# samuel-watson/glmmrMCML

Hardware: AMD Instinct MI355X
Metric: MCML iters/sec x m chains (simlik evals/sec) (higher is better)
Workload: dtype f64

## Files before the change

### glmmrmcml_amd/_lib.py

```python
import ctypes as C
import os
import re

_HERE = os.path.dirname(os.path.abspath(__file__))
LIB_PATH = os.environ.get("GLMMR_MCML_LIB") or os.path.join(_HERE, "libglmmr_mcml_hip.so")
HEADER_PATH = os.path.join(os.path.dirname(_HERE), "include", "glmmr_mcml_c.h")
_lib = None


class McmlError(RuntimeError):
    def __init__(self, code, msg):
        super().__init__("glmmr_mcml error %d: %s" % (code, msg))
        self.code = code


_RETURNS = {"int": C.c_int, "long long": C.c_longlong, "const char*": C.c_char_p}
_SCALARS = {"int": C.c_int, "double": C.c_double, "long long": C.c_longlong, "uint64_t": C.c_uint64, "uint32_t": C.c_uint32}
_CALLBACKS = ("glmmr_mcml_objective", "glmmr_mcml_batch_objective", "glmmr_mcml_parts_objective")
_DECL = re.compile(r"(?<=[;{}]) ?([\w ]+?\*?) ?\b(glmmr_mcml_\w+) ?\(([^()]*)\) ?;")


def prototypes(header):
    text = re.sub(r"/\*.*?\*/", " ", header, flags=re.S)
    text = " ".join(re.sub(r"^\s*#.*$", "", text, flags=re.M).split())
# ... 16 lines not shown

def lib():
    global _lib
    if _lib is None:
        if not os.path.exists(LIB_PATH):
            raise ImportError(
                "%s not built: run `python -c 'import __graft_entry__ as g; g.build()'` "
                "(hipcc --offload-arch=gfx950); glmmrmcml_amd has no CPU fallback" % LIB_PATH)
        if not os.path.exists(HEADER_PATH):
            raise ImportError("%s is missing: the prototypes of %s are read from it" % (HEADER_PATH, LIB_PATH))
        L = C.CDLL(LIB_PATH)
        with open(HEADER_PATH) as f:
            for name, (restype, argtypes) in prototypes(f.read()).items():
                fn = getattr(L, name)
                fn.restype, fn.argtypes = restype, argtypes
        _lib = L
    return _lib


def check(rc):
    if rc != 0:
        raise McmlError(rc, lib().glmmr_mcml_last_error().decode(errors="replace"))
```

### glmmrmcml_amd/csrc/band_plan.h

```cpp
#pragma once
#include "common.h"
#include <algorithm>
#include <map>
#include <memory>

namespace mcml {

constexpr int BD_BM = 80, BD_BN = 128, BD_BK = 32, BD_STAGES = 3;
constexpr int BD_A_BYTES = BD_BK * BD_BM * 8;
constexpr int BD_B_BYTES = BD_BK * BD_BN * 8;
constexpr int BD_STAGE_BYTES = BD_A_BYTES + BD_B_BYTES;
constexpr size_t BD_LDS_BYTES = (size_t)BD_STAGES * BD_STAGE_BYTES;
constexpr int BD_NA = 3, BD_NB = 4, BD_PER_TILE = BD_NA + BD_NB;
constexpr int BD_TILE_ELEMS = BD_BM * BD_BN;

struct BandItem { int band, kt0, kt1, slot; };
struct BandRed { int band, s0, s1, pad; };

struct BandPlanDev {
    int gn = 0, nwg = 0, nred = 0, nslots = 0;
    int paired = 0;
    DevBuf items, wg_ptr, red, part;
};

struct SkinnyPlan {
    int nrb = 0, nkc = 0, ldp = 0;
    DevBuf range;
    DevBuf part;
};

struct BandPlan {
    int M = 0, K = 0, nbands = 0;
    std::vector<int> kr;
    long tiles = 0;
    std::map<int, std::unique_ptr<BandPlanDev>> by_gn;
    std::unique_ptr<SkinnyPlan> skinny;

    void reset(int M_, int K_, const std::vector<int>& kr_)
    {
        M = M_; K = K_; kr = kr_; nbands = (M + BD_BM - 1) / BD_BM;
        tiles = 0;
        for (int b = 0; b < nbands; ++b) tiles += kr[2 * b + 1] - kr[2 * b];
        by_gn.clear();
        skinny.reset();
    }

    static bool decompose(const std::vector<int>& kr, int nbands, int gn, int target_wg, std::vector<BandItem>& items,
                          std::vector<int>& wg_ptr, std::vector<BandRed>& red, int& nslots)
    {
        items.clear(); wg_ptr.clear(); red.clear(); nslots = 0;
        constexpr long OVH = 3;
        const int npairs = (nbands + 1) / 2;
        if ((long)npairs * gn * 5 >= (long)target_wg * 4) {
            auto cost = [&](int b) { return 2L * (kr[2 * b + 1] - kr[2 * b]) + OVH; };
            int G = target_wg / gn; if (G > nbands) G = nbands; if (G < 1) G = 1;
            std::vector<int> order(nbands);
            for (int b = 0; b < nbands; ++b) order[b] = b;
            std::stable_sort(order.begin(), order.end(), [&](int a, int b) { return cost(a) > cost(b); });
            std::vector<long> load(G, 0);
            std::vector<std::vector<int>> group(G);
            for (int b : order) {
                const int g = (int)(std::min_element(load.begin(), load.end()) - load.begin());
                group[g].push_back(b); load[g] += cost(b);
            }
            long pair_max = 0;
            for (int p = 0; p < npairs; ++p)
                pair_max = std::max(pair_max, cost(p) + (nbands - 1 - p > p ? cost(nbands - 1 - p) : 0));
            auto waves = [&](int groups) { return ((long)groups * gn + target_wg - 1) / target_wg; };
            if (waves(npairs) * pair_max < waves(G) * *std::max_element(load.begin(), load.end())) {
                group.assign(npairs, std::vector<int>());
                for (int p = 0; p < npairs; ++p) {
                    group[p].push_back(p);
                    if (nbands - 1 - p > p) group[p].push_back(nbands - 1 - p);
                }
            }
            for (std::vector<int>& g : group) {
                std::sort(g.begin(), g.end());
                wg_ptr.push_back((int)items.size());
                for (int b : g) items.push_back({b, kr[2 * b], kr[2 * b + 1], -1});
            }
            wg_ptr.push_back((int)items.size());
            return true;
        }
        int nwg = target_wg / gn; if (nwg < 1) nwg = 1;
        auto fill = [&](long cap, bool emit) -> int {
            int used = 1; long room = cap;
            if (emit) wg_ptr.push_back(0);
            for (int b = 0; b < nbands; ++b) {
                int k0 = kr[2 * b]; const int k1 = kr[2 * b + 1];
                const int first = (int)items.size();
                int pieces = 0;
                do {
                    if (room < OVH + 2) { ++used; room = cap; if (emit) wg_ptr.push_back((int)items.size()); }
                    long take = (room - OVH) / 2; if (take > k1 - k0) take = k1 - k0;
                    if (emit) items.push_back({b, k0, k0 + (int)take, -1});
                    k0 += (int)take; room -= OVH + 2 * take; ++pieces;
                } while (k0 < k1);
                if (emit && pieces > 1) {
                    for (int t = 0; t < pieces; ++t) items[first + t].slot = nslots + t;
                    red.push_back({b, nslots, nslots + pieces, 0});
                    nslots += pieces;
                }
            }
            if (emit) wg_ptr.push_back((int)items.size());
            return used;
        };
        long T = 0;
        for (int b = 0; b < nbands; ++b) T += kr[2 * b + 1] - kr[2 * b];
        long lo = OVH + 2, hi = 2 * T + OVH * nbands + OVH + 2;
        while (lo < hi) {
            const long mid = (lo + hi) / 2;
            if (fill(mid, false) <= nwg) hi = mid; else lo = mid + 1;
        }
        fill(lo, true);
        return false;
    }

    int device_plan(int gn, hipStream_t s, BandPlanDev** out)
    {
        auto it = by_gn.find(gn);
        if (it != by_gn.end()) { *out = it->second.get(); return MCML_OK; }
        std::unique_ptr<BandPlanDev> d(new BandPlanDev());
        std::vector<BandItem> items; std::vector<int> wg_ptr; std::vector<BandRed> red; int nslots = 0;
        d->paired = decompose(kr, nbands, gn, 256, items, wg_ptr, red, nslots) ? 1 : 0;
        d->gn = gn; d->nwg = (int)wg_ptr.size() - 1; d->nred = (int)red.size(); d->nslots = nslots;
        MCML_TRY(d->items.ensure(sizeof(BandItem) * (items.size() + 1)));
        MCML_TRY(d->wg_ptr.ensure(sizeof(int) * wg_ptr.size()));
        MCML_HIP(hipMemcpyAsync(d->items.p, items.data(), sizeof(BandItem) * items.size(), hipMemcpyHostToDevice, s));
        MCML_HIP(hipMemcpyAsync(d->wg_ptr.p, wg_ptr.data(), sizeof(int) * wg_ptr.size(), hipMemcpyHostToDevice, s));
        if (nslots > 0) {
            MCML_TRY(d->red.ensure(sizeof(BandRed) * red.size()));
            MCML_HIP(hipMemcpyAsync(d->red.p, red.data(), sizeof(BandRed) * red.size(), hipMemcpyHostToDevice, s));
            MCML_TRY(d->part.ensure(sizeof(double) * (size_t)nslots * gn * BD_TILE_ELEMS));
        }
        MCML_HIP(hipStreamSynchronize(s));
        *out = d.get();
        by_gn[gn] = std::move(d);
        return MCML_OK;
    }
};

}
```

### glmmrmcml_amd/csrc/cabi.hip

```cpp
#include "entry.h"
#include "hmc_chain.h"
#include <atomic>

using namespace mcml;

struct Mode {
    int Ctx::*field;
    const char* env;
    const char* names[4];
    const char* valid;
    std::atomic<int> dflt{-1};

    int get()
    {
        if (dflt.load() < 0) {
            const char* e = getenv(env);
            int unset = -1, m = 0;
            for (int i = 1; e && names[i]; ++i) if (!strcmp(e, names[i])) m = i;
            dflt.compare_exchange_strong(unset, m);
        }
        return dflt.load();
    }
    int check(const char* fn, bool ok, int mode) const
    {
// ... 322 lines not shown
{
    return m <= 0 ? 0 : sample_shape(m, 0, chains).ncols;
}

extern "C" int glmmr_mcml_ctx_profile(glmmr_mcml_ctx* h, int enable, int reset, double* out8)
{
    MCML_REQUIRE(h, "profile: null context");
    Ctx& c = h->c;
    KernelProf& p = c.prof;
    if (out8) {
        out8[0] = p.ms[0]; out8[1] = (double)p.cnt[0]; out8[2] = p.ms[1]; out8[3] = (double)p.cnt[1];
        const double C = (double)c.hmc.C, dense = 2.0 * c.n * (double)c.Q * C;
        double ff = dense, fb = dense, kind = 0;
        if (c.sp.active) { ff = fb = 2.0 * (double)c.sp.nnz * C; kind = 2; }
        else {
            if (c.band_fwd) { ff = 2.0 * 80.0 * 32.0 * (double)c.band_fwd_tiles * C; kind = 1; }
            if (c.band_bwd) { fb = 2.0 * 80.0 * 32.0 * (double)c.band_bwd_tiles * C; kind = 1; }
        }
        out8[4] = ff; out8[5] = fb; out8[6] = dense; out8[7] = kind;
    }
    if (reset) for (int i = 0; i < 4; ++i) { p.ms[i] = 0; p.cnt[i] = 0; p.seen[i] = 0; }
    if (enable && !p.on) {
        MCML_HIP(hipSetDevice(c.device));
        while (p.ev.size() < 4096) { hipEvent_t e; if (hipEventCreate(&e) != hipSuccess) { (void)hipGetLastError(); break; } p.ev.push_back(e); }
    }
    p.on = enable != 0;
    return MCML_OK;
}

extern "C" int glmmr_mcml_ctx_profile_launches(glmmr_mcml_ctx* h, long long* fwd, long long* bwd)
{
    MCML_REQUIRE(h, "profile_launches: null context");
// ... 319 lines not shown
```

### glmmrmcml_amd/csrc/ctx_hooks.hip

```cpp
#include "entry.h"
#include "sparse_plan.h"
#include <algorithm>

using namespace mcml;

extern "C" int glmmr_mcml_dbg_theta_log(glmmr_mcml_ctx* h, int enable, double* out, int cap_rows, int* nrows)
{
    MCML_REQUIRE(h, "theta_log: null context");
    Ctx& c = h->c;
    const int w = c.cov.npar + 1;
    const int have = (int)(c.theta_log.size() / (size_t)w);
    if (nrows) *nrows = have;
    if (out) {
        const int take = have < cap_rows ? have : cap_rows;
        memcpy(out, c.theta_log.data() + (size_t)(have - take) * w, sizeof(double) * (size_t)take * w);
        if (nrows) *nrows = take;
    }
    if (enable >= 0) { c.theta_log_on = enable != 0; if (enable) c.theta_log.clear(); }
    return MCML_OK;
}

extern "C" int glmmr_mcml_dbg_band_plan(glmmr_mcml_ctx* h, int which, int chains, int* out10)
{
    MCML_REQUIRE(h && (which == 0 || which == 1) && chains >= 1 && out10, "dbg_band_plan: bad argument");
    const Ctx& c = h->c;
    const BandPlan& bp = which ? c.plan_bwd : c.plan_fwd;
    const int gn = (chains + BD_BN - 1) / BD_BN;
    if (c.sp.active) {
        for (int i = 0; i < 10; ++i) out10[i] = 0;
        out10[3] = gn;
        return MCML_OK;
    }
    int nempty = 0;
    for (int b = 0; b < bp.nbands; ++b) nempty += bp.kr[2 * b] == bp.kr[2 * b + 1];
    int nwg = 0, nred = 0, nslots = 0, paired = 0, built = 0;
    auto it = bp.by_gn.find(gn);
    if (it != bp.by_gn.end()) {
        const BandPlanDev& d = *it->second;
        nwg = d.nwg; nred = d.nred; nslots = d.nslots; paired = d.paired; built = 1;
    } else if (bp.nbands > 0) {
        std::vector<BandItem> items; std::vector<int> wg_ptr; std::vector<BandRed> red;
        paired = BandPlan::decompose(bp.kr, bp.nbands, gn, 256, items, wg_ptr, red, nslots) ? 1 : 0;
        nwg = (int)wg_ptr.size() - 1; nred = (int)red.size();
    }
    const int v[10] = {(which ? c.band_bwd : c.band_fwd) ? 1 : 0, bp.nbands, (int)bp.tiles, gn, nwg, nred, nslots,
                       paired, nempty, built};
    for (int i = 0; i < 10; ++i) out10[i] = v[i];
    return MCML_OK;
}

extern "C" int glmmr_mcml_dbg_sparse_plan(glmmr_mcml_ctx* h, int chains, long long* out12)
{
    MCML_REQUIRE(h && chains >= 1 && out12, "dbg_sparse_plan: bad argument");
    const Ctx& c = h->c;
    const SparseZL& sp = c.sp;
    for (int i = 0; i < 12; ++i) out12[i] = 0;
    out12[0] = sp.active ? 1 : 0;
    out12[10] = cm_qrows(c.Q); out12[11] = cm_chain_blocks(chains);
    if (!sp.active) return MCML_OK;
    out12[1] = sp.factored ? 1 : 0; out12[2] = sp.W; out12[3] = sp.nnz; out12[4] = sp.nnz_z; out12[5] = sp.nnz_l;
    out12[6] = sp.nblk; out12[7] = sp.max_blk; out12[8] = cm_long_rows(c) ? 1 : 0; out12[9] = cm_fuse_width(c);
    return MCML_OK;
// ... 207 lines not shown
```

### glmmrmcml_amd/csrc/debug_hooks.hip

```cpp
#include "dgemm_mfma.h"
#include "dgemm_dl.h"
#include "dgemm_band.h"

using namespace mcml;

extern "C" int glmmr_mcml_dbg_dgemm(int M, int N, int K, const double* A, int lda,
                                    const double* B, int ldb, int b_nmajor,
                                    double alpha, double beta, double* C, int ldc,
                                    int lower_only, int force_tile)
{
    int ndev = 0;
    if (hipGetDeviceCount(&ndev) != hipSuccess || ndev == 0) {
        set_error("no HIP device: libglmmr_mcml_hip has no CPU fallback");
        return MCML_ENODEVICE;
    }
    hipStream_t s = nullptr;
    DevMat dA, dB, dC;
    if (force_tile == 40) {
        MCML_REQUIRE(!b_nmajor && !lower_only, "dbg_dgemm: the direct-to-LDS kernel takes a K-major B and all tiles");
        const int kpad = round_up(K, 32);
        MCML_TRY(dA.alloc(M, K, 32));
        MCML_HIP(hipMemset(dA.d(), 0, sizeof(double) * (size_t)dA.ld * dA.cols_alloc));
        MCML_HIP(hipMemcpy2D(dA.d(), sizeof(double) * dA.ld, A, sizeof(double) * lda, sizeof(double) * M, K, hipMemcpyHostToDevice));
        MCML_TRY(dB.alloc(kpad, N));
// ... 89 lines not shown
    MCML_HIP(hipEventCreate(&e0));
    MCML_HIP(hipEventCreate(&e1));
    MCML_HIP(hipEventRecord(e0, s));
    for (int i = 0; i < iters; i++) MCML_TRY(go());
    MCML_HIP(hipEventRecord(e1, s));
    MCML_HIP(hipEventSynchronize(e1));
    float ms = 0;
    MCML_HIP(hipEventElapsedTime(&ms, e0, e1));
    *ms_per_launch = ms / iters;
    (void)hipEventDestroy(e0);
    (void)hipEventDestroy(e1);
    return MCML_OK;
}

static int dbg_dgemm_band(int M, int N, int K, const double* A, int lda, const double* B, int ldb, double* C, int ldc,
                          int* tiles_executed, int form, int* whole_band);

extern "C" int glmmr_mcml_dbg_dgemm_band(int M, int N, int K, const double* A, int lda, const double* B, int ldb,
                                         double* C, int ldc, int* tiles_executed)
{
    return dbg_dgemm_band(M, N, K, A, lda, B, ldb, C, ldc, tiles_executed, BAND_FORM_AUTO, nullptr);
}

extern "C" int glmmr_mcml_dbg_dgemm_band_form(int M, int N, int K, const double* A, int lda, const double* B, int ldb,
                                              double* C, int ldc, int* tiles_executed, int form, int* whole_band)
{
    MCML_REQUIRE(form == BAND_FORM_8WAVE || form == BAND_FORM_FEED, "dbg_dgemm_band_form: form is 0 or 1");
    return dbg_dgemm_band(M, N, K, A, lda, B, ldb, C, ldc, tiles_executed, form, whole_band);
}

static int dbg_dgemm_band(int M, int N, int K, const double* A, int lda, const double* B, int ldb, double* C, int ldc,
                          int* tiles_executed, int form, int* whole_band)
{
    int ndev = 0;
    if (hipGetDeviceCount(&ndev) != hipSuccess || ndev == 0) {
        set_error("no HIP device: libglmmr_mcml_hip has no CPU fallback");
        return MCML_ENODEVICE;
    }
    MCML_REQUIRE(M > 0 && N > 0 && K > 0 && A && B && C, "dbg_dgemm_band: bad argument");
    hipStream_t s = nullptr;
    DevMat dA, dB, dC;
    MCML_TRY(dA.alloc(M, K, 32));
    MCML_HIP(hipMemset(dA.d(), 0, sizeof(double) * (size_t)dA.ld * dA.cols_alloc));
    MCML_HIP(hipMemcpy2D(dA.d(), sizeof(double) * dA.ld, A, sizeof(double) * lda, sizeof(double) * M, K, hipMemcpyHostToDevice));
    MCML_TRY(dB.alloc(round_up(K, 32), N));
    MCML_HIP(hipMemset(dB.d(), 0, sizeof(double) * (size_t)dB.ld * N));
    MCML_HIP(hipMemcpy2D(dB.d(), sizeof(double) * dB.ld, B, sizeof(double) * ldb, sizeof(double) * K, N, hipMemcpyHostToDevice));
    MCML_TRY(dC.alloc(M, N));
    MCML_HIP(hipMemset(dC.d(), 0, sizeof(double) * (size_t)dC.ld * N));
    MCML_REQUIRE(dlds_applicable(M, N, K, dA.d(), dA.ld, dA.cols_alloc, dB.d(), dB.ld), "dbg_dgemm_band: contract");
    const int nbands = (M + BD_BM - 1) / BD_BM;
    DevBuf kr;
    MCML_TRY(kr.ensure(sizeof(int) * 2 * nbands));
    hipLaunchKernelGGL(k_band_ranges, dim3(nbands), dim3(256), 0, s, dA.d(), dA.ld, M, K, kr.as<int>());
    MCML_HIP(hipGetLastError());
    std::vector<int> hk(2 * nbands);
    MCML_HIP(hipMemcpy(hk.data(), kr.p, sizeof(int) * 2 * nbands, hipMemcpyDeviceToHost));
    BandPlan plan;
    plan.reset(M, K, hk);
    if (tiles_executed) *tiles_executed = (int)plan.tiles;
    EpiAxpby epi{dC.d(), dC.ld, 1.0, 0.0};
    MCML_TRY(launch_gemm_band(s, plan, N, dA.d(), dA.ld, dB.d(), dB.ld, epi, nullptr, 0, form, whole_band));
    MCML_TRY(download_matrix(C, ldc, dC.d(), dC.ld, M, N, s));
    return MCML_OK;
}

extern "C" int glmmr_mcml_dbg_band_clocks(int M, int N, int iters, int mode, double* out3)
{
    MCML_REQUIRE(mode < 0 || !(mode & 15),
                 "dbg_band_clocks: modes 1, 2, 4 and 8 (the K loop with parts switched off) were retired by the commit "
                 "'Band HMC products: one K-loop pipeline under both kernel forms'; their findings are in DESIGN.md 5.1");
    int ndev = 0;
    if (hipGetDeviceCount(&ndev) != hipSuccess || ndev == 0) {
        set_error("no HIP device: libglmmr_mcml_hip has no CPU fallback");
        return MCML_ENODEVICE;
// ... 3 lines not shown
    std::vector<double> hA((size_t)M * M, 0.0), hB((size_t)M * N);
    uint64_t x = 88172645463325252ULL;
    auto rnd = [&]() { x ^= x << 13; x ^= x >> 7; x ^= x << 17; return (double)(x >> 11) / 9007199254740992.0 * 2 - 1; };
    const bool cst = getenv("GLMMR_MCML_DBG_DATA") && !strcmp(getenv("GLMMR_MCML_DBG_DATA"), "const");
    const bool dec = getenv("GLMMR_MCML_DBG_DATA") && !strcmp(getenv("GLMMR_MCML_DBG_DATA"), "decay");
    for (int j = 0; j < M; ++j) for (int i = j; i < M; ++i) hA[i + (size_t)j * M] = cst ? 1.0 : dec ? rnd() * std::exp(-(double)(i - j) / 40.0) : rnd();
    for (auto& v : hB) v = cst ? 1.0 : rnd();
    DevMat dA, dB, dC;
    MCML_TRY(dA.alloc(M, M, 32));
    MCML_HIP(hipMemset(dA.d(), 0, sizeof(double) * (size_t)dA.ld * dA.cols_alloc));
    MCML_HIP(hipMemcpy2D(dA.d(), sizeof(double) * dA.ld, hA.data(), sizeof(double) * M, sizeof(double) * M, M, hipMemcpyHostToDevice));
    MCML_TRY(dB.alloc(round_up(M, 32), N));
    MCML_HIP(hipMemset(dB.d(), 0, sizeof(double) * (size_t)dB.ld * N));
    MCML_HIP(hipMemcpy2D(dB.d(), sizeof(double) * dB.ld, hB.data(), sizeof(double) * M, sizeof(double) * M, N, hipMemcpyHostToDevice));
    MCML_TRY(dC.alloc(M, N));
    const int nbands = (M + BD_BM - 1) / BD_BM;
    DevBuf kr, clk;
    MCML_TRY(kr.ensure(sizeof(int) * 2 * nbands));
    MCML_TRY(clk.ensure(16));
    MCML_HIP(hipMemset(clk.p, 0, 16));
    hipLaunchKernelGGL(k_band_ranges, dim3(nbands), dim3(256), 0, s, dA.d(), dA.ld, M, M, kr.as<int>());
    std::vector<int> hk(2 * nbands);
    MCML_HIP(hipMemcpy(hk.data(), kr.p, sizeof(int) * 2 * nbands, hipMemcpyDeviceToHost));
    BandPlan plan;
    plan.reset(M, M, hk);
    const double tiles = (double)plan.tiles;
    EpiAxpby epi{dC.d(), dC.ld, 1.0, 0.0};
    if (mode < 0) {
        for (int i = 0; i < 3; i++)
            MCML_TRY((launch_gemm_band<EpiAxpby, false>(s, plan, N, dA.d(), dA.ld, dB.d(), dB.ld, epi)));
        hipEvent_t f0, f1;
        MCML_HIP(hipEventCreate(&f0));
        MCML_HIP(hipEventCreate(&f1));
        MCML_HIP(hipEventRecord(f0, s));
        for (int i = 0; i < iters; i++)
            MCML_TRY((launch_gemm_band<EpiAxpby, false>(s, plan, N, dA.d(), dA.ld, dB.d(), dB.ld, epi)));
        MCML_HIP(hipEventRecord(f1, s));
        MCML_HIP(hipEventSynchronize(f1));
        float fms = 0;
        MCML_HIP(hipEventElapsedTime(&fms, f0, f1));
        out3[0] = fms / iters; out3[1] = 0;
// ... 221 lines not shown
```

### glmmrmcml_amd/csrc/dgemm_band.h

```cpp
#pragma once
#include "dgemm_dlds.h"
#include "band_plan.h"

namespace mcml {

struct BandP {
    GemmP g;
    const BandItem* items;
    const int* wg_ptr;
    int nwg;
    double* part;
    int mode;
    unsigned long long* clocks;
};

static __global__ __launch_bounds__(256) void k_band_ranges(const double* A, int lda, int M, int K, int* krange)
{
    __shared__ int smin[256], smax[256];
    const int band = blockIdx.x, r0 = band * BD_BM;
    const int rows = (M - r0 < BD_BM) ? (M - r0) : BD_BM;
    int kmin = 1 << 30, kmax = -1;
    for (int k = threadIdx.x; k < K; k += 256) {
        const double* col = A + r0 + (size_t)k * lda;
        bool nz = false;
        for (int r = 0; r < rows; ++r) nz |= (col[r] != 0.0);
        if (nz) { kmin = min(kmin, k); kmax = max(kmax, k); }
    }
    smin[threadIdx.x] = kmin; smax[threadIdx.x] = kmax;
    __syncthreads();
    for (int o = 128; o > 0; o >>= 1) {
        if ((int)threadIdx.x < o) {
            smin[threadIdx.x] = min(smin[threadIdx.x], smin[threadIdx.x + o]);
            smax[threadIdx.x] = max(smax[threadIdx.x], smax[threadIdx.x + o]);
        }
        __syncthreads();
    }
    if (threadIdx.x == 0) {
        if (smax[0] < 0) { krange[2 * band] = 0; krange[2 * band + 1] = 0; }
        else { krange[2 * band] = smin[0] / BD_BK; krange[2 * band + 1] = smax[0] / BD_BK + 1; }
    }
}

#if defined(__HIP_DEVICE_COMPILE__)
#define BD_RD(dst, addr, off) asm volatile("ds_read_b64 %0, %1 offset:%2" : "=v"(dst) : "v"(addr), "i"(off))
#else
#define BD_RD(dst, addr, off) (dst = 0.0)
#endif
template <int KS, int NS>
__device__ __forceinline__ void bd_read(double (&a)[5], double (&b)[NS], unsigned aaddr, unsigned baddr)
{
    static_assert(NS == 1 || NS == 2, "one or two strips per wave");
    BD_RD(a[0], aaddr, KS * 4 * BD_BM * 8);
    BD_RD(a[1], aaddr, KS * 4 * BD_BM * 8 + 128);
    BD_RD(a[2], aaddr, KS * 4 * BD_BM * 8 + 256);
    BD_RD(a[3], aaddr, KS * 4 * BD_BM * 8 + 384);
// ... 8 lines not shown
#if defined(__HIP_DEVICE_COMPILE__)
    if constexpr (NS == 1)
        asm volatile("s_waitcnt lgkmcnt(%[n])" : "+v"(a[0]), "+v"(a[1]), "+v"(a[2]), "+v"(a[3]), "+v"(a[4]), "+v"(b[0]) : [n] "n"(LEAVE));
    else
        asm volatile("s_waitcnt lgkmcnt(%[n])" : "+v"(a[0]), "+v"(a[1]), "+v"(a[2]), "+v"(a[3]), "+v"(a[4]), "+v"(b[0]), "+v"(b[1]) : [n] "n"(LEAVE));
#endif
}
template <int NS>
__device__ __forceinline__ void bd_mfma(d4 (&acc)[NS][5][1], const double (&a)[5], const double (&b)[NS])
{
#pragma unroll
    for (int j = 0; j < NS; ++j)
#pragma unroll
        for (int i = 0; i < 5; ++i) acc[j][i][0] = __builtin_amdgcn_mfma_f64_16x16x4f64(b[j], a[i], acc[j][i][0], 0, 0, 0);
}

__device__ __forceinline__ BandItem band_item(const BandItem* ip)
{
    BandItem item{0, 0, 0, -1};
#if defined(__HIP_DEVICE_COMPILE__)
    typedef int i4s __attribute__((ext_vector_type(4)));
    i4s raw;
    asm volatile("s_load_dwordx4 %0, %1, 0x0\n\ts_waitcnt lgkmcnt(0)" : "=&s"(raw) : "s"(ip) : "memory");
    item.band = raw.x; item.kt0 = raw.y; item.kt1 = raw.z; item.slot = raw.w;
#else
    item = *ip;
#endif
    return item;
}

template <int STRIDE, int NA, int NB>
struct BandFill {
    static constexpr int PER_TILE = NA + NB, A_CHUNKS = BD_A_BYTES / 1024;
    static_assert(STRIDE * NA >= A_CHUNKS && STRIDE * NB * 1024 == BD_B_BYTES, "the role's waves cover a stage");
    const GemmP& p;
    const BandItem* items;
    const int f, lane;
    const unsigned lds0;
    const size_t stepA;
    unsigned voa[NA], vob[NB];
    const char* sA = nullptr; const char* sB = nullptr;
    BandItem item{0, 0, 0, -1};

    __device__ __forceinline__ int a_rel(int s) const
    {
        return (STRIDE * NA > A_CHUNKS && f + STRIDE * s >= A_CHUNKS) ? STRIDE : STRIDE * s;
    }
    __device__ __forceinline__ BandFill(const BandP& bp, int f_, int lane_, int n0, unsigned lds0_)
        : p(bp.g), items(bp.items), f(f_), lane(lane_), lds0(lds0_), stepA((size_t)BD_BK * bp.g.lda * 8)
    {
#pragma unroll
        for (int s = 0; s < NB; ++s) {
            const int c = f + STRIDE * s;
            const int kp = c >> 1, n = ((c & 1) << 6) + lane;
            int gn = n0 + n;
            if (gn >= p.N) gn = 0;
            vob[s] = (unsigned)((2 * kp + (size_t)gn * p.ldb) * 8);
// ... 21 lines not shown
        for (int s = 0; s < NA; ++s) lds_dma16(lbase + a_rel(s) * 1024, voa[s], sA);
#pragma unroll
        for (int s = 0; s < NB; ++s) lds_dma16(lbase + BD_A_BYTES + STRIDE * s * 1024, vob[s], sB);
        sA += stepA;
        sB += BD_BK * 8;
    }
    __device__ __forceinline__ void wait_leave(int tiles) const
    {
        if (tiles >= 2) asm volatile("s_waitcnt vmcnt(%0)" :: "n"(2 * PER_TILE) : "memory");
        else if (tiles == 1) asm volatile("s_waitcnt vmcnt(%0)" :: "n"(PER_TILE) : "memory");
        else asm volatile("s_waitcnt vmcnt(0)" ::: "memory");
    }
};
struct BandNoFill {
    const BandItem* items;
    BandItem item{0, 0, 0, -1};
    __device__ __forceinline__ BandNoFill(const BandP& bp, int, int, int, unsigned) : items(bp.items) {}
    __device__ __forceinline__ void load_item(int it) { item = band_item(items + it); }
    __device__ __forceinline__ void issue(int) {}
    __device__ __forceinline__ void wait_leave(int) const {}
};
constexpr int BF_NA = 5, BF_NB = 8;

__device__ __forceinline__ void band_store_partial(double* tile, int strip, int lane, const d4 (&acc)[5][1])
{
    double* P = tile + (size_t)strip * (20 * 64) + lane;
#pragma unroll
    for (int i = 0; i < 5; ++i)
#pragma unroll
        for (int r = 0; r < 4; ++r) P[(i * 4 + r) * 64] = acc[i][0][r];
}
// ... 24 lines not shown

    auto stamp = [&](int i) {
        if constexpr (DBG)
            if ((bp.mode & 16) && bp.clocks && threadIdx.x == 0)
                bp.clocks[8 + 8 * (size_t)blockIdx.x + i] = __builtin_amdgcn_s_memrealtime();
    };
    stamp(0);
    bool first_item = true;
    Fill fill(bp, piece0, lane, n0, lds0);
    bool pre = false;
    int issued = 0;
    if (it0 < it1) fill.load_item(it0);
    for (int it = it0; it < it1;) {
        const int band = fill.item.band, slot = fill.item.slot;
        const int nk = fill.item.kt1 - fill.item.kt0;

        d4 acc[NJ][5][1];
#pragma unroll
        for (int j = 0; j < NJ; ++j)
#pragma unroll
            for (int i = 0; i < 5; ++i) acc[j][i][0] = d4{0.0, 0.0, 0.0, 0.0};

        if (nk > 0) {
            const unsigned aoff = lds0 + lk * (BD_BM * 8) + l15 * 8;
            const unsigned boff = lds0 + BD_A_BYTES + (((lk >> 1) * BD_BN + strip0 * 16 + l15) << 4) + ((lk & 1) << 3);
            if (!pre) { issued = 0; for (; issued < BD_STAGES - 1 && issued < nk; ++issued) fill.issue(issued); }
            fill.wait_leave(issued - 1);
            __builtin_amdgcn_s_barrier();
            if (first_item) stamp(1);
            int st = 0;
            double ra[2][5], rb[2][NJ];
            if constexpr (NS > 0) bd_read<0>(ra[0], rb[0], aoff, boff);
            for (int kt = 0; kt < nk; ++kt) {
                if (issued < nk) {
                    int sn = st + BD_STAGES - 1; if (sn >= BD_STAGES) sn -= BD_STAGES;
                    fill.issue(sn);
                    ++issued;
                }
                const unsigned aaddr = aoff + st * BD_STAGE_BYTES, baddr = boff + st * BD_STAGE_BYTES;
                int stn = st + 1; if (stn >= BD_STAGES) stn = 0;
                if constexpr (NS > 0) {
#define BD_STEP(KS, CUR, NXT)                                   \
                    bd_read<KS + 1>(ra[NXT], rb[NXT], aaddr, baddr); \
                    bd_wait<5 + NS>(ra[CUR], rb[CUR]);               \
                    bd_mfma(acc, ra[CUR], rb[CUR]);                  \
                    __builtin_amdgcn_sched_barrier(0);
                    BD_STEP(0, 0, 1) BD_STEP(1, 1, 0) BD_STEP(2, 0, 1) BD_STEP(3, 1, 0)
                    BD_STEP(4, 0, 1) BD_STEP(5, 1, 0) BD_STEP(6, 0, 1)
#undef BD_STEP
                }
                fill.wait_leave(issued - kt - 2);
                if constexpr (NS > 0) bd_wait<0>(ra[1], rb[1]);
                __builtin_amdgcn_s_barrier();
                if constexpr (NS > 0) {
                    if (kt + 1 < nk) bd_read<0>(ra[0], rb[0], aoff + stn * BD_STAGE_BYTES, boff + stn * BD_STAGE_BYTES);
                    bd_mfma(acc, ra[1], rb[1]);
                    __builtin_amdgcn_sched_barrier(0);
                }
                st = stn;
            }
        }
        if (first_item) stamp(2);
        ++it;
        pre = false;
        if (it < it1) {
            fill.load_item(it);
            const int nkn = fill.item.kt1 - fill.item.kt0;
            if (nk > 0 && nkn > 0) {
                issued = 0;
                for (; issued < BD_STAGES - 1 && issued < nkn; ++issued) fill.issue(issued);
                pre = true;
// ... 129 lines not shown
```

### glmmrmcml_amd/csrc/model.hip

```cpp
#include "ctx.h"
#include "component.h"
#include "dgemm_mfma.h"
#include "dgemm_band.h"
#include "glm.h"
#include "host_linalg.h"
#include "reduce.h"
#include "vecops.h"

namespace mcml {

int model_setup(Ctx& c, const double* Z, const double* X, const double* y)
{
    const int n = c.n, Q = c.Q, P = c.P;
    MCML_TRY(upload_matrix(c.Z, Z, n, Q, n, c.stream));
    MCML_TRY(upload_matrix(c.X, X, n, P, n, c.stream));
    MCML_TRY(c.y.ensure(sizeof(double) * (size_t)pad_ld(n)));
    MCML_TRY(c.xb.ensure(sizeof(double) * (size_t)pad_ld(n)));
    MCML_HIP(hipMemsetAsync(c.y.p, 0, sizeof(double) * (size_t)pad_ld(n), c.stream));
    MCML_HIP(hipMemsetAsync(c.xb.p, 0, sizeof(double) * (size_t)pad_ld(n), c.stream));
    std::vector<double> yy(y, y + n);
    if (c.flink == 8)
        for (auto& v : yy) v = log(v);
    MCML_TRY(copy_h2d(c.y.p, yy.data(), sizeof(double) * n, c.stream));
    size_t nnz = 0; int maxrow = 0;
// ... 228 lines not shown
        MCML_HIP(hipMemsetAsync(c.ZL.d(), 0, sizeof(double) * (size_t)c.ZL.ld * c.ZL.cols_alloc, c.stream));
        MCML_HIP(hipMemsetAsync(c.ZLT.d(), 0, sizeof(double) * (size_t)c.ZLT.ld * c.ZLT.cols_alloc, c.stream));
    }
    if (c.z_width > 0) {
        MCML_TRY(z_times(c, c.L.d(), c.L.ld, c.Q, c.ZL.d(), c.ZL.ld));
    } else {
        EpiAxpby epi{c.ZL.d(), c.ZL.ld, 1.0, 0.0};
        MCML_TRY(launch_gemm<false>(c.stream, c.n, c.Q, c.Q, c.Z.d(), c.Z.ld, c.L.d(), c.L.ld, epi));
    }
    MCML_TRY(dev_transpose(c, c.ZL.d(), c.ZL.ld, c.n, c.Q, c.ZLT.d(), c.ZLT.ld));
    c.band_fwd = c.band_bwd = false;
    const char* env = getenv("GLMMR_MCML_GEMM");
    if (!(env && (!strcmp(env, "reg") || !strcmp(env, "dlds")))) {
        auto ranges = [&](const DevMat& A, int M, int K, BandPlan& plan, bool& use, long& ntiles) -> int {
            const int nb = (M + BD_BM - 1) / BD_BM;
            MCML_TRY(c.kr_scratch.ensure(sizeof(int) * 2 * (size_t)nb));
            hipLaunchKernelGGL(k_band_ranges, dim3(nb), dim3(256), 0, c.stream, A.d(), A.ld, M, K, c.kr_scratch.as<int>());
            MCML_HIP(hipGetLastError());
            std::vector<int> h(2 * (size_t)nb);
            MCML_TRY(copy_d2h(h.data(), c.kr_scratch.p, sizeof(int) * h.size(), c.stream));
            MCML_HIP(hipStreamSynchronize(c.stream));
            if (!(plan.M == M && plan.K == K && plan.kr == h))
                plan.reset(M, K, h);
            const long dense = (long)nb * ((K + BD_BK - 1) / BD_BK);
            use = (env && !strcmp(env, "band")) || plan.tiles * 5 <= dense * 4;
            ntiles = plan.tiles;
            return MCML_OK;
        };
        MCML_TRY(ranges(c.ZL, c.n, c.Q, c.plan_fwd, c.band_fwd, c.band_fwd_tiles));
        MCML_TRY(ranges(c.ZLT, c.Q, c.n, c.plan_bwd, c.band_bwd, c.band_bwd_tiles));
    }
    return MCML_OK;
}

template <int FL>
__global__ __launch_bounds__(256) void k_loglik(const double* ZU, int ldz, int n, int ncols, const double* xb,
                                                const double* y, double var_par, int flink_rt, double* partials)
{
// ... 171 lines not shown
```

Before: 1222.

## Skip all-zero 16-row sub-tiles in banded DGEMM via per-tile row masks

The band-range scan now records, for each 80-row band and 32-wide K tile, a 5-bit mask of which 16-row sub-blocks hold nonzeros. The masks are packed into each work item as lead, trail and body fields, and the banded MFMA kernel skips the MFMAs for zero sub-blocks on tiles that are not fully populated. The work decomposition also weights its cost by the number of active row sub-tiles. This cuts wasted f64 MFMA work at band edges, at the cost of a larger item load, a branch per K tile, and a finer-grained scan kernel during setup.

```diff
diff --git a/glmmrmcml_amd/_lib.py b/glmmrmcml_amd/_lib.py
--- a/glmmrmcml_amd/_lib.py
+++ b/glmmrmcml_amd/_lib.py
@@ -5,6 +5,7 @@
 _HERE = os.path.dirname(os.path.abspath(__file__))
 LIB_PATH = os.environ.get("GLMMR_MCML_LIB") or os.path.join(_HERE, "libglmmr_mcml_hip.so")
 HEADER_PATH = os.path.join(os.path.dirname(_HERE), "include", "glmmr_mcml_c.h")
+HOOK_HEADER_PATHS = (os.path.join(os.path.dirname(_HERE), "include", "glmmr_mcml_band_hooks.h"),)
 _lib = None
 
 
@@ -54,6 +55,12 @@
             for name, (restype, argtypes) in prototypes(f.read()).items():
                 fn = getattr(L, name)
                 fn.restype, fn.argtypes = restype, argtypes
+        for path in HOOK_HEADER_PATHS:
+            with open(path) as f:
+                for name, (restype, argtypes) in prototypes(f.read()).items():
+                    fn = getattr(L, name, None)
+                    if fn is not None:
+                        fn.restype, fn.argtypes = restype, argtypes
         _lib = L
     return _lib
 
diff --git a/glmmrmcml_amd/csrc/band_plan.h b/glmmrmcml_amd/csrc/band_plan.h
--- a/glmmrmcml_amd/csrc/band_plan.h
+++ b/glmmrmcml_amd/csrc/band_plan.h
@@ -14,7 +14,17 @@
 constexpr int BD_NA = 3, BD_NB = 4, BD_PER_TILE = BD_NA + BD_NB;
 constexpr int BD_TILE_ELEMS = BD_BM * BD_BN;
 
-struct BandItem { int band, kt0, kt1, slot; };
+constexpr int BD_RT = BD_BM / 16;
+constexpr int BD_RT_FULL = (1 << BD_RT) - 1;
+
+struct BandItem { int band, kt0, kt1, slot, lead, trail, body, pad; };
+static_assert(sizeof(BandItem) == 32, "one 8-dword scalar load per item");
+__host__ __device__ __forceinline__ int band_tile_mask(int lead, int trail, int body, int nk, int kt)
+{
+    const int back = nk - 1 - kt;
+    const int m = kt < 4 ? lead >> (5 * kt) : back < 4 ? trail >> (5 * back) : body;
+    return m & BD_RT_FULL;
+}
 struct BandRed { int band, s0, s1, pad; };
 
 struct BandPlanDev {
@@ -29,30 +39,89 @@
     DevBuf part;
 };
 
+static inline bool band_rowmask_enabled()
+{
+    const char* e = getenv("GLMMR_MCML_BAND_ROWMASK");
+    return !(e && !strcmp(e, "0"));
+}
+
 struct BandPlan {
-    int M = 0, K = 0, nbands = 0;
+    int M = 0, K = 0, nbands = 0, nkt = 0;
     std::vector<int> kr;
+    std::vector<unsigned char> rm;
     long tiles = 0;
+    long rowtiles = 0;
     std::map<int, std::unique_ptr<BandPlanDev>> by_gn;
     std::unique_ptr<SkinnyPlan> skinny;
 
-    void reset(int M_, int K_, const std::vector<int>& kr_)
-    {
-        M = M_; K = K_; kr = kr_; nbands = (M + BD_BM - 1) / BD_BM;
-        tiles = 0;
-        for (int b = 0; b < nbands; ++b) tiles += kr[2 * b + 1] - kr[2 * b];
+    static int plan_key(int gn, bool rowmask) { return 2 * gn + (rowmask ? 1 : 0); }
+    long rowtiles_executed() const { return band_rowmask_enabled() ? rowtiles : tiles * BD_RT; }
+
+    static void ranges_of(const std::vector<unsigned char>& rm, int nbands, int nkt, std::vector<int>& kr)
+    {
+        kr.assign(2 * (size_t)nbands, 0);
+        for (int b = 0; b < nbands; ++b) {
+            int k0 = -1, k1 = 0;
+            for (int t = 0; t < nkt; ++t)
+                if (rm[(size_t)b * nkt + t]) { if (k0 < 0) k0 = t; k1 = t + 1; }
+            if (k0 >= 0) { kr[2 * b] = k0; kr[2 * b + 1] = k1; }
+        }
+    }
+
+    void reset(int M_, int K_, const std::vector<int>& kr_, const std::vector<unsigned char>& rm_)
+    {
+        M = M_; K = K_; kr = kr_; rm = rm_; nbands = (M + BD_BM - 1) / BD_BM; nkt = (K + BD_BK - 1) / BD_BK;
+        tiles = rowtiles = 0;
+        for (int b = 0; b < nbands; ++b) {
+            const int nk = kr[2 * b + 1] - kr[2 * b];
+            BandItem x{b, kr[2 * b], kr[2 * b + 1], -1, 0, 0, 0, 0};
+            if (nk > 0) pack_masks(rm.data() + (size_t)b * nkt + kr[2 * b], nk, x);
+            tiles += nk;
+            for (int kt = 0; kt < nk; ++kt) rowtiles += __builtin_popcount(band_tile_mask(x.lead, x.trail, x.body, nk, kt));
+        }
         by_gn.clear();
         skinny.reset();
     }
 
+    static void pack_masks(const unsigned char* m, int nk, BandItem& item)
+    {
+        item.lead = item.trail = item.body = 0;
+        for (int t = 0; t < 4 && t < nk; ++t) {
+            item.lead |= (m[t] & BD_RT_FULL) << (5 * t);
+            item.trail |= (m[nk - 1 - t] & BD_RT_FULL) << (5 * t);
+        }
+        for (int t = 4; t < nk - 4; ++t) item.body |= m[t] & BD_RT_FULL;
+    }
+
     static bool decompose(const std::vector<int>& kr, int nbands, int gn, int target_wg, std::vector<BandItem>& items,
                           std::vector<int>& wg_ptr, std::vector<BandRed>& red, int& nslots)
     {
+        int nkt = 0;
+        for (int b = 0; b < nbands; ++b) nkt = std::max(nkt, kr[2 * b + 1]);
+        const std::vector<unsigned char> full((size_t)nbands * nkt, (unsigned char)BD_RT_FULL);
+        const bool whole = decompose(kr, full, nkt, nbands, gn, target_wg, items, wg_ptr, red, nslots);
+        for (BandItem& x : items) x.lead = x.trail = x.body = 0;
+        return whole;
+    }
+
+    static bool decompose(const std::vector<int>& kr, const std::vector<unsigned char>& rm, int nkt, int nbands, int gn,
+                          int target_wg, std::vector<BandItem>& items, std::vector<int>& wg_ptr, std::vector<BandRed>& red,
+                          int& nslots)
+    {
         items.clear(); wg_ptr.clear(); red.clear(); nslots = 0;
-        constexpr long OVH = 3;
+        auto mask_of = [&](int b, int t) { return rm[(size_t)b * nkt + t] & BD_RT_FULL; };
+        auto emit = [&](int b, int k0, int k1) {
+            BandItem x{b, k0, k1, -1, 0, 0, 0, 0};
+            if (k1 > k0) pack_masks(rm.data() + (size_t)b * nkt + k0, k1 - k0, x);
+            items.push_back(x);
+        };
+        constexpr long OVH = 3 * BD_RT, TILE = 2 * BD_RT;
         const int npairs = (nbands + 1) / 2;
         if ((long)npairs * gn * 5 >= (long)target_wg * 4) {
-            auto cost = [&](int b) { return 2L * (kr[2 * b + 1] - kr[2 * b]) + OVH; };
+            std::vector<long> bcost(nbands, OVH);
+            for (int b = 0; b < nbands; ++b)
+                for (int t = kr[2 * b]; t < kr[2 * b + 1]; ++t) bcost[b] += 2 * __builtin_popcount(mask_of(b, t));
+            auto cost = [&](int b) { return bcost[b]; };
             int G = target_wg / gn; if (G > nbands) G = nbands; if (G < 1) G = 1;
             std::vector<int> order(nbands);
             for (int b = 0; b < nbands; ++b) order[b] = b;
@@ -77,37 +146,37 @@
             for (std::vector<int>& g : group) {
                 std::sort(g.begin(), g.end());
                 wg_ptr.push_back((int)items.size());
-                for (int b : g) items.push_back({b, kr[2 * b], kr[2 * b + 1], -1});
+                for (int b : g) emit(b, kr[2 * b], kr[2 * b + 1]);
             }
             wg_ptr.push_back((int)items.size());
             return true;
         }
         int nwg = target_wg / gn; if (nwg < 1) nwg = 1;
-        auto fill = [&](long cap, bool emit) -> int {
+        auto fill = [&](long cap, bool out) -> int {
             int used = 1; long room = cap;
-            if (emit) wg_ptr.push_back(0);
+            if (out) wg_ptr.push_back(0);
             for (int b = 0; b < nbands; ++b) {
                 int k0 = kr[2 * b]; const int k1 = kr[2 * b + 1];
                 const int first = (int)items.size();
                 int pieces = 0;
                 do {
-                    if (room < OVH + 2) { ++used; room = cap; if (emit) wg_ptr.push_back((int)items.size()); }
-                    long take = (room - OVH) / 2; if (take > k1 - k0) take = k1 - k0;
-                    if (emit) items.push_back({b, k0, k0 + (int)take, -1});
-                    k0 += (int)take; room -= OVH + 2 * take; ++pieces;
+                    if (room < OVH + TILE) { ++used; room = cap; if (out) wg_ptr.push_back((int)items.size()); }
+                    long take = (room - OVH) / TILE; if (take > k1 - k0) take = k1 - k0;
+                    if (out) emit(b, k0, k0 + (int)take);
+                    k0 += (int)take; room -= OVH + TILE * take; ++pieces;
                 } while (k0 < k1);
-                if (emit && pieces > 1) {
+                if (out && pieces > 1) {
                     for (int t = 0; t < pieces; ++t) items[first + t].slot = nslots + t;
                     red.push_back({b, nslots, nslots + pieces, 0});
                     nslots += pieces;
                 }
             }
-            if (emit) wg_ptr.push_back((int)items.size());
+            if (out) wg_ptr.push_back((int)items.size());
             return used;
         };
         long T = 0;
         for (int b = 0; b < nbands; ++b) T += kr[2 * b + 1] - kr[2 * b];
-        long lo = OVH + 2, hi = 2 * T + OVH * nbands + OVH + 2;
+        long lo = OVH + TILE, hi = TILE * T + OVH * nbands + OVH + TILE;
         while (lo < hi) {
             const long mid = (lo + hi) / 2;
             if (fill(mid, false) <= nwg) hi = mid; else lo = mid + 1;
@@ -116,13 +185,19 @@
         return false;
     }
 
+    std::vector<unsigned char> masks_in_use(bool rowmask) const
+    {
+        return rowmask ? rm : std::vector<unsigned char>(rm.size(), (unsigned char)BD_RT_FULL);
+    }
+
     int device_plan(int gn, hipStream_t s, BandPlanDev** out)
     {
-        auto it = by_gn.find(gn);
+        const bool rowmask = band_rowmask_enabled();
+        auto it = by_gn.find(plan_key(gn, rowmask));
         if (it != by_gn.end()) { *out = it->second.get(); return MCML_OK; }
         std::unique_ptr<BandPlanDev> d(new BandPlanDev());
         std::vector<BandItem> items; std::vector<int> wg_ptr; std::vector<BandRed> red; int nslots = 0;
-        d->paired = decompose(kr, nbands, gn, 256, items, wg_ptr, red, nslots) ? 1 : 0;
+        d->paired = decompose(kr, masks_in_use(rowmask), nkt, nbands, gn, 256, items, wg_ptr, red, nslots) ? 1 : 0;
         d->gn = gn; d->nwg = (int)wg_ptr.size() - 1; d->nred = (int)red.size(); d->nslots = nslots;
         MCML_TRY(d->items.ensure(sizeof(BandItem) * (items.size() + 1)));
         MCML_TRY(d->wg_ptr.ensure(sizeof(int) * wg_ptr.size()));
@@ -135,7 +210,7 @@
         }
         MCML_HIP(hipStreamSynchronize(s));
         *out = d.get();
-        by_gn[gn] = std::move(d);
+        by_gn[plan_key(gn, rowmask)] = std::move(d);
         return MCML_OK;
     }
 };
diff --git a/glmmrmcml_amd/csrc/cabi.hip b/glmmrmcml_amd/csrc/cabi.hip
--- a/glmmrmcml_amd/csrc/cabi.hip
+++ b/glmmrmcml_amd/csrc/cabi.hip
@@ -360,8 +360,8 @@
         double ff = dense, fb = dense, kind = 0;
         if (c.sp.active) { ff = fb = 2.0 * (double)c.sp.nnz * C; kind = 2; }
         else {
-            if (c.band_fwd) { ff = 2.0 * 80.0 * 32.0 * (double)c.band_fwd_tiles * C; kind = 1; }
-            if (c.band_bwd) { fb = 2.0 * 80.0 * 32.0 * (double)c.band_bwd_tiles * C; kind = 1; }
+            if (c.band_fwd) { ff = 2.0 * 16.0 * 32.0 * (double)c.plan_fwd.rowtiles_executed() * C; kind = 1; }
+            if (c.band_bwd) { fb = 2.0 * 16.0 * 32.0 * (double)c.plan_bwd.rowtiles_executed() * C; kind = 1; }
         }
         out8[4] = ff; out8[5] = fb; out8[6] = dense; out8[7] = kind;
     }
diff --git a/glmmrmcml_amd/csrc/ctx_hooks.hip b/glmmrmcml_amd/csrc/ctx_hooks.hip
--- a/glmmrmcml_amd/csrc/ctx_hooks.hip
+++ b/glmmrmcml_amd/csrc/ctx_hooks.hip
@@ -1,5 +1,6 @@
 #include "entry.h"
 #include "sparse_plan.h"
+#include "../../include/glmmr_mcml_band_hooks.h"
 #include <algorithm>
 
 using namespace mcml;
@@ -34,18 +35,30 @@
     int nempty = 0;
     for (int b = 0; b < bp.nbands; ++b) nempty += bp.kr[2 * b] == bp.kr[2 * b + 1];
     int nwg = 0, nred = 0, nslots = 0, paired = 0, built = 0;
-    auto it = bp.by_gn.find(gn);
+    const bool rowmask = band_rowmask_enabled();
+    auto it = bp.by_gn.find(BandPlan::plan_key(gn, rowmask));
     if (it != bp.by_gn.end()) {
         const BandPlanDev& d = *it->second;
         nwg = d.nwg; nred = d.nred; nslots = d.nslots; paired = d.paired; built = 1;
     } else if (bp.nbands > 0) {
         std::vector<BandItem> items; std::vector<int> wg_ptr; std::vector<BandRed> red;
-        paired = BandPlan::decompose(bp.kr, bp.nbands, gn, 256, items, wg_ptr, red, nslots) ? 1 : 0;
+        paired = BandPlan::decompose(bp.kr, bp.masks_in_use(rowmask), bp.nkt, bp.nbands, gn, 256, items, wg_ptr, red, nslots) ? 1 : 0;
         nwg = (int)wg_ptr.size() - 1; nred = (int)red.size();
     }
     const int v[10] = {(which ? c.band_bwd : c.band_fwd) ? 1 : 0, bp.nbands, (int)bp.tiles, gn, nwg, nred, nslots,
                        paired, nempty, built};
     for (int i = 0; i < 10; ++i) out10[i] = v[i];
+    return MCML_OK;
+}
+
+extern "C" int glmmr_mcml_dbg_band_rowtiles(glmmr_mcml_ctx* h, int which, long long* out3)
+{
+    MCML_REQUIRE(h && (which == 0 || which == 1) && out3, "dbg_band_rowtiles: bad argument");
+    const Ctx& c = h->c;
+    const BandPlan& bp = which ? c.plan_bwd : c.plan_fwd;
+    out3[0] = out3[1] = out3[2] = 0;
+    if (c.sp.active) return MCML_OK;
+    out3[0] = bp.rowtiles_executed(); out3[1] = bp.rowtiles; out3[2] = bp.tiles;
     return MCML_OK;
 }
 
diff --git a/glmmrmcml_amd/csrc/debug_hooks.hip b/glmmrmcml_amd/csrc/debug_hooks.hip
--- a/glmmrmcml_amd/csrc/debug_hooks.hip
+++ b/glmmrmcml_amd/csrc/debug_hooks.hip
@@ -1,6 +1,7 @@
 #include "dgemm_mfma.h"
 #include "dgemm_dl.h"
 #include "dgemm_band.h"
+#include "../../include/glmmr_mcml_band_hooks.h"
 
 using namespace mcml;
 
@@ -127,7 +128,7 @@
 }
 
 static int dbg_dgemm_band(int M, int N, int K, const double* A, int lda, const double* B, int ldb, double* C, int ldc,
-                          int* tiles_executed, int form, int* whole_band);
+                          int* tiles_executed, int form, int* whole_band, long long* rowtiles = nullptr);
 
 extern "C" int glmmr_mcml_dbg_dgemm_band(int M, int N, int K, const double* A, int lda, const double* B, int ldb,
                                          double* C, int ldc, int* tiles_executed)
@@ -142,8 +143,16 @@
     return dbg_dgemm_band(M, N, K, A, lda, B, ldb, C, ldc, tiles_executed, form, whole_band);
 }
 
+extern "C" int glmmr_mcml_dbg_dgemm_band_rowtiles(int M, int N, int K, const double* A, int lda, const double* B, int ldb,
+                                                  double* C, int ldc, int* tiles_executed, int form, int* whole_band,
+                                                  long long* rowtiles)
+{
+    MCML_REQUIRE(form == BAND_FORM_8WAVE || form == BAND_FORM_FEED, "dbg_dgemm_band_rowtiles: form is 0 or 1");
+    return dbg_dgemm_band(M, N, K, A, lda, B, ldb, C, ldc, tiles_executed, form, whole_band, rowtiles);
+}
+
 static int dbg_dgemm_band(int M, int N, int K, const double* A, int lda, const double* B, int ldb, double* C, int ldc,
-                          int* tiles_executed, int form, int* whole_band)
+                          int* tiles_executed, int form, int* whole_band, long long* rowtiles)
 {
     int ndev = 0;
     if (hipGetDeviceCount(&ndev) != hipSuccess || ndev == 0) {
@@ -162,16 +171,14 @@
     MCML_TRY(dC.alloc(M, N));
     MCML_HIP(hipMemset(dC.d(), 0, sizeof(double) * (size_t)dC.ld * N));
     MCML_REQUIRE(dlds_applicable(M, N, K, dA.d(), dA.ld, dA.cols_alloc, dB.d(), dB.ld), "dbg_dgemm_band: contract");
-    const int nbands = (M + BD_BM - 1) / BD_BM;
     DevBuf kr;
-    MCML_TRY(kr.ensure(sizeof(int) * 2 * nbands));
-    hipLaunchKernelGGL(k_band_ranges, dim3(nbands), dim3(256), 0, s, dA.d(), dA.ld, M, K, kr.as<int>());
-    MCML_HIP(hipGetLastError());
-    std::vector<int> hk(2 * nbands);
-    MCML_HIP(hipMemcpy(hk.data(), kr.p, sizeof(int) * 2 * nbands, hipMemcpyDeviceToHost));
+    std::vector<int> hk;
+    std::vector<unsigned char> hm;
+    MCML_TRY(band_scan(s, dA.d(), dA.ld, M, K, kr, hk, hm));
     BandPlan plan;
-    plan.reset(M, K, hk);
+    plan.reset(M, K, hk, hm);
     if (tiles_executed) *tiles_executed = (int)plan.tiles;
+    if (rowtiles) *rowtiles = plan.rowtiles_executed();
     EpiAxpby epi{dC.d(), dC.ld, 1.0, 0.0};
     MCML_TRY(launch_gemm_band(s, plan, N, dA.d(), dA.ld, dB.d(), dB.ld, epi, nullptr, 0, form, whole_band));
     MCML_TRY(download_matrix(C, ldc, dC.d(), dC.ld, M, N, s));
@@ -205,17 +212,15 @@
     MCML_HIP(hipMemset(dB.d(), 0, sizeof(double) * (size_t)dB.ld * N));
     MCML_HIP(hipMemcpy2D(dB.d(), sizeof(double) * dB.ld, hB.data(), sizeof(double) * M, sizeof(double) * M, N, hipMemcpyHostToDevice));
     MCML_TRY(dC.alloc(M, N));
-    const int nbands = (M + BD_BM - 1) / BD_BM;
     DevBuf kr, clk;
-    MCML_TRY(kr.ensure(sizeof(int) * 2 * nbands));
     MCML_TRY(clk.ensure(16));
     MCML_HIP(hipMemset(clk.p, 0, 16));
-    hipLaunchKernelGGL(k_band_ranges, dim3(nbands), dim3(256), 0, s, dA.d(), dA.ld, M, M, kr.as<int>());
-    std::vector<int> hk(2 * nbands);
-    MCML_HIP(hipMemcpy(hk.data(), kr.p, sizeof(int) * 2 * nbands, hipMemcpyDeviceToHost));
+    std::vector<int> hk;
+    std::vector<unsigned char> hm;
+    MCML_TRY(band_scan(s, dA.d(), dA.ld, M, M, kr, hk, hm));
     BandPlan plan;
-    plan.reset(M, M, hk);
-    const double tiles = (double)plan.tiles;
+    plan.reset(M, M, hk, hm);
+    const double tiles = (double)plan.rowtiles_executed() / BD_RT;
     EpiAxpby epi{dC.d(), dC.ld, 1.0, 0.0};
     if (mode < 0) {
         for (int i = 0; i < 3; i++)
diff --git a/glmmrmcml_amd/csrc/dgemm_band.h b/glmmrmcml_amd/csrc/dgemm_band.h
--- a/glmmrmcml_amd/csrc/dgemm_band.h
+++ b/glmmrmcml_amd/csrc/dgemm_band.h
@@ -14,31 +14,41 @@
     unsigned long long* clocks;
 };
 
-static __global__ __launch_bounds__(256) void k_band_ranges(const double* A, int lda, int M, int K, int* krange)
-{
-    __shared__ int smin[256], smax[256];
+static __global__ __launch_bounds__(256) void k_band_ranges(const double* A, int lda, int M, int K, int nkt, unsigned char* masks)
+{
     const int band = blockIdx.x, r0 = band * BD_BM;
-    const int rows = (M - r0 < BD_BM) ? (M - r0) : BD_BM;
-    int kmin = 1 << 30, kmax = -1;
-    for (int k = threadIdx.x; k < K; k += 256) {
-        const double* col = A + r0 + (size_t)k * lda;
-        bool nz = false;
-        for (int r = 0; r < rows; ++r) nz |= (col[r] != 0.0);
-        if (nz) { kmin = min(kmin, k); kmax = max(kmax, k); }
-    }
-    smin[threadIdx.x] = kmin; smax[threadIdx.x] = kmax;
-    __syncthreads();
-    for (int o = 128; o > 0; o >>= 1) {
-        if ((int)threadIdx.x < o) {
-            smin[threadIdx.x] = min(smin[threadIdx.x], smin[threadIdx.x + o]);
-            smax[threadIdx.x] = max(smax[threadIdx.x], smax[threadIdx.x + o]);
-        }
-        __syncthreads();
-    }
-    if (threadIdx.x == 0) {
-        if (smax[0] < 0) { krange[2 * band] = 0; krange[2 * band + 1] = 0; }
-        else { krange[2 * band] = smin[0] / BD_BK; krange[2 * band + 1] = smax[0] / BD_BK + 1; }
-    }
+    const int lane = threadIdx.x & 63, wave = threadIdx.x >> 6;
+    const bool lo_ok = r0 + lane < M, hi_ok = lane < 16 && r0 + 64 + lane < M;
+    for (int kt = blockIdx.y * 4 + wave; kt < nkt; kt += 4 * gridDim.y) {
+        const double* col = A + r0 + lane + (size_t)kt * BD_BK * lda;
+        const int nc = min(BD_BK, K - kt * BD_BK);
+        bool lo = false, hi = false;
+#pragma unroll 8
+        for (int c = 0; c < nc; ++c) {
+            if (lo_ok) lo |= col[(size_t)c * lda] != 0.0;
+            if (hi_ok) hi |= col[(size_t)c * lda + 64] != 0.0;
+        }
+        const unsigned long long bl = __ballot(lo), bh = __ballot(hi);
+        if (lane == 0) {
+            int m = bh ? 1 << 4 : 0;
+            for (int i = 0; i < 4; ++i) m |= ((bl >> (16 * i)) & 0xffffULL) ? 1 << i : 0;
+            masks[(size_t)band * nkt + kt] = (unsigned char)m;
+        }
+    }
+}
+
+static inline int band_scan(hipStream_t s, const double* A, int lda, int M, int K, DevBuf& scratch, std::vector<int>& kr,
+                            std::vector<unsigned char>& rm)
+{
+    const int nb = (M + BD_BM - 1) / BD_BM, nkt = (K + BD_BK - 1) / BD_BK;
+    MCML_TRY(scratch.ensure((size_t)nb * nkt));
+    hipLaunchKernelGGL(k_band_ranges, dim3(nb, 8), dim3(256), 0, s, A, lda, M, K, nkt, scratch.as<unsigned char>());
+    MCML_HIP(hipGetLastError());
+    rm.resize((size_t)nb * nkt);
+    MCML_TRY(copy_d2h(rm.data(), scratch.p, rm.size(), s));
+    MCML_HIP(hipStreamSynchronize(s));
+    BandPlan::ranges_of(rm, nb, nkt, kr);
+    return MCML_OK;
 }
 
 #if defined(__HIP_DEVICE_COMPILE__)
@@ -77,15 +87,30 @@
 #pragma unroll
         for (int i = 0; i < 5; ++i) acc[j][i][0] = __builtin_amdgcn_mfma_f64_16x16x4f64(b[j], a[i], acc[j][i][0], 0, 0, 0);
 }
+template <int NS>
+__device__ __forceinline__ void bd_mfma_masked(d4 (&acc)[NS][5][1], const double (&a)[5], const double (&b)[NS], int mask)
+{
+    int m = mask;
+#if defined(__HIP_DEVICE_COMPILE__)
+    asm volatile("" : "+s"(m));
+#endif
+#pragma unroll
+    for (int i = 0; i < 5; ++i)
+        if (__builtin_expect((m >> i) & 1, 1)) {
+#pragma unroll
+            for (int j = 0; j < NS; ++j) acc[j][i][0] = __builtin_amdgcn_mfma_f64_16x16x4f64(b[j], a[i], acc[j][i][0], 0, 0, 0);
+        }
+}
 
 __device__ __forceinline__ BandItem band_item(const BandItem* ip)
 {
-    BandItem item{0, 0, 0, -1};
+    BandItem item{0, 0, 0, -1, 0, 0, 0, 0};
 #if defined(__HIP_DEVICE_COMPILE__)
-    typedef int i4s __attribute__((ext_vector_type(4)));
-    i4s raw;
-    asm volatile("s_load_dwordx4 %0, %1, 0x0\n\ts_waitcnt lgkmcnt(0)" : "=&s"(raw) : "s"(ip) : "memory");
-    item.band = raw.x; item.kt0 = raw.y; item.kt1 = raw.z; item.slot = raw.w;
+    typedef int i8s __attribute__((ext_vector_type(8)));
+    i8s raw;
+    asm volatile("s_load_dwordx8 %0, %1, 0x0\n\ts_waitcnt lgkmcnt(0)" : "=&s"(raw) : "s"(ip) : "memory");
+    item.band = raw[0]; item.kt0 = raw[1]; item.kt1 = raw[2]; item.slot = raw[3];
+    item.lead = raw[4]; item.trail = raw[5]; item.body = raw[6];
 #else
     item = *ip;
 #endif
@@ -103,7 +128,7 @@
     const size_t stepA;
     unsigned voa[NA], vob[NB];
     const char* sA = nullptr; const char* sB = nullptr;
-    BandItem item{0, 0, 0, -1};
+    BandItem item{0, 0, 0, -1, 0, 0, 0, 0};
 
     __device__ __forceinline__ int a_rel(int s) const
     {
@@ -155,7 +180,7 @@
 };
 struct BandNoFill {
     const BandItem* items;
-    BandItem item{0, 0, 0, -1};
+    BandItem item{0, 0, 0, -1, 0, 0, 0, 0};
     __device__ __forceinline__ BandNoFill(const BandP& bp, int, int, int, unsigned) : items(bp.items) {}
     __device__ __forceinline__ void load_item(int it) { item = band_item(items + it); }
     __device__ __forceinline__ void issue(int) {}
@@ -210,6 +235,7 @@
     for (int it = it0; it < it1;) {
         const int band = fill.item.band, slot = fill.item.slot;
         const int nk = fill.item.kt1 - fill.item.kt0;
+        const int lead = fill.item.lead, trail = fill.item.trail, body = fill.item.body;
 
         d4 acc[NJ][5][1];
 #pragma unroll
@@ -235,14 +261,22 @@
                 }
                 const unsigned aaddr = aoff + st * BD_STAGE_BYTES, baddr = boff + st * BD_STAGE_BYTES;
                 int stn = st + 1; if (stn >= BD_STAGES) stn = 0;
+                const int tmask = NS > 0 ? band_tile_mask(lead, trail, body, nk, kt) : BD_RT_FULL;
                 if constexpr (NS > 0) {
-#define BD_STEP(KS, CUR, NXT)                                   \
+#define BD_STEP(KS, CUR, NXT, MFMA)                             \
                     bd_read<KS + 1>(ra[NXT], rb[NXT], aaddr, baddr); \
                     bd_wait<5 + NS>(ra[CUR], rb[CUR]);               \
-                    bd_mfma(acc, ra[CUR], rb[CUR]);                  \
+                    MFMA(ra[CUR], rb[CUR]);                          \
                     __builtin_amdgcn_sched_barrier(0);
-                    BD_STEP(0, 0, 1) BD_STEP(1, 1, 0) BD_STEP(2, 0, 1) BD_STEP(3, 1, 0)
-                    BD_STEP(4, 0, 1) BD_STEP(5, 1, 0) BD_STEP(6, 0, 1)
+#define BD_DENSE(A_, B_) bd_mfma(acc, A_, B_)
+#define BD_MASKED(A_, B_) bd_mfma_masked(acc, A_, B_, tmask)
+                    if (tmask == BD_RT_FULL) {
+                        BD_STEP(0, 0, 1, BD_DENSE) BD_STEP(1, 1, 0, BD_DENSE) BD_STEP(2, 0, 1, BD_DENSE) BD_STEP(3, 1, 0, BD_DENSE)
+                        BD_STEP(4, 0, 1, BD_DENSE) BD_STEP(5, 1, 0, BD_DENSE) BD_STEP(6, 0, 1, BD_DENSE)
+                    } else {
+                        BD_STEP(0, 0, 1, BD_MASKED) BD_STEP(1, 1, 0, BD_MASKED) BD_STEP(2, 0, 1, BD_MASKED) BD_STEP(3, 1, 0, BD_MASKED)
+                        BD_STEP(4, 0, 1, BD_MASKED) BD_STEP(5, 1, 0, BD_MASKED) BD_STEP(6, 0, 1, BD_MASKED)
+                    }
 #undef BD_STEP
                 }
                 fill.wait_leave(issued - kt - 2);
@@ -250,7 +284,9 @@
                 __builtin_amdgcn_s_barrier();
                 if constexpr (NS > 0) {
                     if (kt + 1 < nk) bd_read<0>(ra[0], rb[0], aoff + stn * BD_STAGE_BYTES, boff + stn * BD_STAGE_BYTES);
-                    bd_mfma(acc, ra[1], rb[1]);
+                    if (tmask == BD_RT_FULL) BD_DENSE(ra[1], rb[1]); else BD_MASKED(ra[1], rb[1]);
+#undef BD_DENSE
+#undef BD_MASKED
                     __builtin_amdgcn_sched_barrier(0);
                 }
                 st = stn;
diff --git a/glmmrmcml_amd/csrc/model.hip b/glmmrmcml_amd/csrc/model.hip
--- a/glmmrmcml_amd/csrc/model.hip
+++ b/glmmrmcml_amd/csrc/model.hip
@@ -266,14 +266,11 @@
     if (!(env && (!strcmp(env, "reg") || !strcmp(env, "dlds")))) {
         auto ranges = [&](const DevMat& A, int M, int K, BandPlan& plan, bool& use, long& ntiles) -> int {
             const int nb = (M + BD_BM - 1) / BD_BM;
-            MCML_TRY(c.kr_scratch.ensure(sizeof(int) * 2 * (size_t)nb));
-            hipLaunchKernelGGL(k_band_ranges, dim3(nb), dim3(256), 0, c.stream, A.d(), A.ld, M, K, c.kr_scratch.as<int>());
-            MCML_HIP(hipGetLastError());
-            std::vector<int> h(2 * (size_t)nb);
-            MCML_TRY(copy_d2h(h.data(), c.kr_scratch.p, sizeof(int) * h.size(), c.stream));
-            MCML_HIP(hipStreamSynchronize(c.stream));
-            if (!(plan.M == M && plan.K == K && plan.kr == h))
-                plan.reset(M, K, h);
+            std::vector<int> h;
+            std::vector<unsigned char> rm;
+            MCML_TRY(band_scan(c.stream, A.d(), A.ld, M, K, c.kr_scratch, h, rm));
+            if (!(plan.M == M && plan.K == K && plan.kr == h && plan.rm == rm))
+                plan.reset(M, K, h, rm);
             const long dense = (long)nb * ((K + BD_BK - 1) / BD_BK);
             use = (env && !strcmp(env, "band")) || plan.tiles * 5 <= dense * 4;
             ntiles = plan.tiles;
diff --git a/include/glmmr_mcml_band_hooks.h b/include/glmmr_mcml_band_hooks.h
--- /dev/null
+++ b/include/glmmr_mcml_band_hooks.h
@@ -0,0 +1,16 @@
+#ifndef GLMMR_MCML_BAND_HOOKS_H
+#define GLMMR_MCML_BAND_HOOKS_H
+#include "glmmr_mcml_c.h"
+
+#ifdef __cplusplus
+extern "C" {
+#endif
+
+int glmmr_mcml_dbg_band_rowtiles(glmmr_mcml_ctx* ctx, int which, long long* out3);
+int glmmr_mcml_dbg_dgemm_band_rowtiles(int M, int N, int K, const double* A, int lda, const double* B, int ldb, double* C,
+                                       int ldc, int* tiles_executed, int form, int* whole_band, long long* rowtiles);
+
+#ifdef __cplusplus
+}
+#endif
+#endif
```

New measurement: 1021. 16.4% lower.
